# vmanam0451/distributed-path-tracer

Measured on AMD Instinct MI355X. Metric: Msamples/sec, Cornell box 1920x1080, 256 spp per frame, 8 bounces (camera paths traced per second), higher is better.
Workload: dtype f32

## Files before the change

distributed-path-tracer_amd/__init__.py:

```python
import atexit
import ctypes as C
import os
import re
import weakref

import numpy as np

_HERE = os.path.dirname(os.path.abspath(__file__))
LIB_PATH = os.environ.get("PTX_LIB") or os.path.join(_HERE, "libptx_hip.so")
HEADER_PATH = os.path.join(os.path.dirname(_HERE), "include", "ptx.h")

OK, ERR_INVALID, ERR_IO, ERR_PARSE, ERR_NO_CAMERA, ERR_NO_DEVICE, ERR_HIP, ERR_UNSUPPORTED = range(8)
NO_SUN_LIGHT = 0xFFFFFFFF

(ARR_MODEL_XFORM, ARR_MODEL_AABB, ARR_MODEL_SURF, ARR_SURF_RANGE, ARR_MESH_AABB, ARR_VERTICES, ARR_TRIANGLES,
 ARR_MATERIALS, ARR_KD_NODES, ARR_KD_REFS, ARR_CAMERA, ARR_SUN, ARR_MODEL_NAMES, ARR_TEXTURES, ARR_TEXELS, ARR_SURF_TEX, ARR_TEXELS_F32,
 ARR_LIGHT_TRIS, ARR_LIGHT_CDF, ARR_LIGHT_GEOM) = range(20)


class PtxError(RuntimeError):
    def __init__(self, code, msg):
        super().__init__(f"ptx error {code}: {msg}")
        self.code = code


class WorkItem(C.Structure):
    _fields_ = [("mesh_name", C.c_char_p), ("primitives", C.POINTER(C.c_int32)), ("n_primitives", C.c_uint32)]


class LoadOpts(C.Structure):
    _fields_ = [("camera_index", C.c_uint32), ("sun_light_index", C.c_uint32), ("filter_primitives", C.c_uint32),
                ("n_work", C.c_uint32), ("work", C.POINTER(WorkItem))]
# ... 217 lines not shown
    EXACT_MATH_FORMS = ("rcp", "sqrt", "rsqrt")

    def exact_math_check(self):
        out = np.zeros(len(self.EXACT_MATH_FORMS), np.uint64)
        _check(lib().ptx_exact_math_check(self.h, out.ctypes.data))
        return {n: int(v) for n, v in zip(self.EXACT_MATH_FORMS, out)}

    def leaf_intersect(self, corners, rays, refs=None, leaf_ordered=False):
        c = np.ascontiguousarray(corners, np.float32).reshape(-1, 9)
        r = np.ascontiguousarray(rays, np.float32).reshape(-1, 7)
        p = None if refs is None else np.ascontiguousarray(refs, np.uint32)
        if p is not None and p.shape != (len(c),):
            raise ValueError("refs must hold one reference per triangle")
        out = np.zeros((len(r), 3), np.float32)
        tri = np.full(len(r), -1, np.int32)
        _check(lib().ptx_leaf_intersect_batch(self.h, c.ctypes.data, len(c), None if p is None else p.ctypes.data, int(bool(leaf_ordered)),
                                              r.ctypes.data, len(r), out.ctypes.data, tri.ctypes.data))
        return {"t": out[:, 0].copy(), "beta": out[:, 1].copy(), "gamma": out[:, 2].copy(), "triangle": tri}

    def tonemap_encode(self, accum, W, H, spp, out=None):
        ret = out if out is not None else np.zeros((H, W, 4), np.uint8)
        _check(lib().ptx_tonemap_encode(self.h, _ptr(accum), W, H, spp, _ptr(ret)))
        return ret

    def denoise(self, a, b, albedo_cov, normal_depth, spp_a, spp_b, iterations=0, sigma_l=0, sigma_n=0, sigma_z=0, out=None, want_stats=True):
        bufs = [a, b, albedo_cov, normal_depth] + ([out] if out is not None else [])
        shape = tuple(a.shape)
        if len(shape) != 3 or shape[2] != 4 or any(tuple(x.shape) != shape for x in bufs):
            raise ValueError(f"denoise: every buffer must be [H, W, 4] of one size, got {[tuple(x.shape) for x in bufs]}")
        if out is None:
            out = np.empty(shape, np.float32) if isinstance(a, np.ndarray) else a.new_empty(shape)
# ... 29 lines not shown
            lib().ptx_ctx_destroy(self.h)
            self.h = None

    def __del__(self):
        try:
            self.close()
        except Exception:
            pass


_ARR_DTYPE = {ARR_MODEL_XFORM: (np.float32, 12), ARR_MODEL_AABB: (np.float32, 6), ARR_MODEL_SURF: (np.int32, 2),
              ARR_SURF_RANGE: (np.int32, 8), ARR_MESH_AABB: (np.float32, 6), ARR_VERTICES: (np.float32, 11),
              ARR_TRIANGLES: (np.uint32, 3), ARR_MATERIALS: (np.float32, 11), ARR_KD_NODES: (np.uint32, 2),
              ARR_KD_REFS: (np.uint32, 1), ARR_CAMERA: (np.float32, 1), ARR_SUN: (np.float32, 1),
              ARR_TEXTURES: (np.uint32, 4), ARR_TEXELS: (np.uint8, 1), ARR_SURF_TEX: (np.int32, 7), ARR_TEXELS_F32: (np.float32, 1),
              ARR_LIGHT_TRIS: (np.uint32, 2), ARR_LIGHT_CDF: (np.float32, 1), ARR_LIGHT_GEOM: (np.float32, 4)}


class Scene:

    def __init__(self, handle, ctx):
        self.h = handle
        self.ctx = ctx
        _live.add(self)

    @classmethod
    def load_gltf(cls, ctx, path, camera_index=0, sun_light_index=0, work=None):
        h = C.c_void_p()
        opts = LoadOpts(camera_index, sun_light_index, 0, 0, None)
        keep = []
        if work is not None:
# ... 281 lines not shown
```

distributed-path-tracer_amd/csrc/device_core.hpp:

```cpp
#pragma once
#include <hip/hip_runtime.h>
#include <stdint.h>
#include <stdlib.h>
#include <stdio.h>

#include "kernels.hpp"

namespace ptx {

#define DEV __device__ __forceinline__

#ifdef PTX_PROF
struct Prof { uint32_t t[kProfRegions], l[kProfRegions]; };
#define PROF_ARG , Prof& prof
#define PROF_PASS , prof
#define PROF(k) do { const uint64_t m_ = __ballot(true); prof.l[k] += 1u; prof.t[k] += ((threadIdx.x & 63u) == (uint32_t)(__ffsll((long long)m_) - 1)) ? 1u : 0u; } while (0)
#else
#define PROF_ARG
#define PROF_PASS
#define PROF(k) do { } while (0)
#endif

constexpr float kEps = 0.0001f;
constexpr double kPi = 3.14159265358979323846;
// ... 144 lines not shown
	if ((X.x > X.y) | (Y.x > Y.y) | (Z.x > Z.y)) return false;
	const f2 tx = (X - bc(o.x)) * bc(inv.x), ty = (Y - bc(o.y)) * bc(inv.y), tz = (Z - bc(o.z)) * bc(inv.z);
	const f2 sm = (tx + ty) + tz;
	const float s = sm.x + sm.y;
	if (s == s) {
		nr = hw_max3(hw_min(tx.x, tx.y), hw_min(ty.x, ty.y), hw_min(tz.x, tz.y));
		fr = hw_min3(hw_max(tx.x, tx.y), hw_max(ty.x, ty.y), hw_max(tz.x, tz.y));
	} else {
		nr = pmax(pmax(pmin(tx.x, tx.y), pmin(ty.x, ty.y)), pmin(tz.x, tz.y));
		fr = pmin(pmin(pmax(tx.x, tx.y), pmax(ty.x, ty.y)), pmax(tz.x, tz.y));
	}
	if (nr > fr) return false;
	return fr >= 0;
}

template <int PB>
DEV bool mesh_traverse(const Geom& g, uint32_t root, float nr, float fr, V3 o, V3 d, MeshHit& out, const Spill& spill PROF_ARG) {
	PROF(PB);
	const PRay pr = pack_ray(o, d);
	int sp = 0;
	uint32_t n0 = 0, n1 = 0, n2 = 0;
	float m0 = 0, m1 = 0, m2 = 0;
	uint32_t node = root;
	float min_dist = nr, max_dist = fr;
	bool have = true;
	for (;;) {
		PROF(PB + 1);
		if (!have) {
			if (sp == 0) return false;
			sp--;
// ... 42 lines not shown
				max_dist = split_dist;
			}
			if (!has_next) { valid = false; break; }
			node = next;
#ifdef PTX_LDS_PAIR_FETCH
			nd = pair_fetch ? (next == li ? kid0 : kid1) : g.nodes[node];
#else
			nd = (pair_fetch && g.pair) ? (next == li ? kid0 : kid1) : g.nodes[node];
#endif
		}
		if (!valid) continue;
		uint32_t first_ref = nd.x, count = nd.y >> 2;
		float best_t = -1.0f, bb1 = 0, bb2 = 0;
		uint32_t best_tri = 0;
		uint32_t key = 0;
		for (uint32_t i = 0; i < count; i++) {
			PROF(PB + 3);
			const uint32_t slot = g.leaf_ordered ? first_ref + i : g.refs[first_ref + i];
			const float4 r0 = g.tris[3 * slot], r1 = g.tris[3 * slot + 1], r2 = g.tris[3 * slot + 2];
			const uint32_t ti = __float_as_uint(r2.z);
			float be, ga;
			const float t = tri_test_pk<true>(r0, r1, make_float2(r2.x, r2.y), pr, be, ga, key);
			if (t >= 0 && t <= max_dist && (t < best_t || !(best_t >= 0))) { best_t = t; bb1 = be; bb2 = ga; best_tri = ti; }
		}
		if (key >= kRcpKeyEnd) {
			best_t = -1.0f; bb1 = 0; bb2 = 0; best_tri = 0;
			for (uint32_t i = 0; i < count; i++) {
				const uint32_t slot = g.leaf_ordered ? first_ref + i : g.refs[first_ref + i];
				const float4 r0 = g.tris[3 * slot], r1 = g.tris[3 * slot + 1], r2 = g.tris[3 * slot + 2];
				float be, ga;
				const float t = tri_test_pk<false>(r0, r1, make_float2(r2.x, r2.y), pr, be, ga, key);
				if (t >= 0 && t <= max_dist && (t < best_t || !(best_t >= 0))) { best_t = t; bb1 = be; bb2 = ga; best_tri = __float_as_uint(r2.z); }
			}
		}
		if (!(best_t >= 0)) continue;
		out.t = best_t; out.b1 = bb1; out.b2 = bb2; out.tri = best_tri;
		return true;
	}
}

template <int MODE, int PB>
DEV bool mesh_traverse_m(const Geoms& G, const SurfaceRec& sf, float nr, float fr, V3 o, V3 d, MeshHit& out, const Spill& spill PROF_ARG) {
	if constexpr (MODE == MODE_GLOBAL) return mesh_traverse<PB>(G.glb, sf.kd_root, nr, fr, o, d, out, spill PROF_PASS);
	else if constexpr (MODE == MODE_LDS) return mesh_traverse<PB>(G.lds, sf.lds_root, nr, fr, o, d, out, spill PROF_PASS);
	else {
		if (sf.lds_root != 0xFFFFFFFFu) return mesh_traverse<PB>(G.lds, sf.lds_root, nr, fr, o, d, out, spill PROF_PASS);
		return mesh_traverse<PB>(G.glb, sf.kd_root, nr, fr, o, d, out, spill PROF_PASS);
	}
}
template <int MODE, int PB>
DEV bool mesh_intersect_m(const Geoms& G, const SurfaceRec& sf, V3 o, V3 d, V3 inv, MeshHit& out, const Spill& spill PROF_ARG) {
	float nr, fr;
	if (!aabb_test_inv(sf.bmin, sf.bmax, o, inv, nr, fr)) return false;
	return mesh_traverse_m<MODE, PB>(G, sf, nr, fr, o, d, out, spill PROF_PASS);
}

struct SceneHit { float dist; int surface; uint32_t tri; float b1, b2; };

template <int MODE>
DEV bool scene_traverse(const DevScene& S, const Geoms& g, V3 o, V3 d, SceneHit& best, const Spill& spill) {
#ifdef PTX_PROF
// ... 519 lines not shown
```

distributed-path-tracer_amd/csrc/flat_scene.hpp:

```cpp
#pragma once
#include <cstdint>
#include <vector>
#include <string>

namespace ptx {

struct KdNode { uint32_t w0, w1; };
constexpr uint32_t KD_LEAF = 3u;
inline KdNode kd_make_branch(float split, uint32_t axis, bool has_l, bool has_r, uint32_t first_child) {
	uint32_t bits;
	__builtin_memcpy(&bits, &split, 4);
	return {bits, axis | (has_l ? 4u : 0u) | (has_r ? 8u : 0u) | (first_child << 4)};
}
inline KdNode kd_make_leaf(uint32_t first_ref, uint32_t count) { return {first_ref, KD_LEAF | (count << 2)}; }

struct TriRec { float ax, ay, az; uint32_t ia; float bx, by, bz; uint32_t ib; float cx, cy, cz; uint32_t ic; };

struct TriIsect { float e2y, e1z, e2z, e1y; float e1x, e2x, ay, az; float ax, c3, p0, p1; };
TriIsect make_tri_isect(const float* a, const float* b, const float* c, uint32_t gid);

struct HitRec { float a[3], ua, b[3], ub, c[3], uc, na[3], va, nb[3], vb, nc[3], vc, ta[3], p0, tb[3], p1, tc[3], p2; };
static_assert(sizeof(HitRec) == 144, "HitRec layout");

struct ModelRec {
// ... 8 lines not shown
	float pad0;
	float box[6], pbox[6];
};
static_assert(sizeof(ModelRec) == 60 * 4, "ModelRec layout");

struct SurfaceRec {
	float bmin[3], bmax[3];
	uint32_t kd_root;
	uint32_t tri_base;
	uint32_t lds_root;
	uint32_t model;
	float pbmin[3], pbmax[3];
	float box[6], pbox[6];
};
static_assert(sizeof(SurfaceRec) == 28 * 4, "SurfaceRec layout");
template <class Rec> inline void interleave_boxes(Rec& r) {
	for (int k = 0; k < 3; k++) { r.box[2 * k] = r.bmin[k]; r.box[2 * k + 1] = r.bmax[k]; r.pbox[2 * k] = r.pbmin[k]; r.pbox[2 * k + 1] = r.pbmax[k]; }
}

struct MaterialRec {
	float albedo[3]; float opacity;
	float emissive[3]; float roughness;
	float metallic; float ior; uint32_t shadow_catcher; uint32_t tex_mask;
	int32_t tex[7];
	int32_t pad;
};
static_assert(sizeof(MaterialRec) == 80, "MaterialRec layout");

struct TexRec { uint32_t w, h, c_srgb , offset ; };
constexpr uint32_t kTexSrgb = 1u << 8, kTexFloat = 1u << 16;
// ... 45 lines not shown
	SunRec sun{};
	uint32_t kd_max_depth = 0;
	bool any_texture = false;
	bool any_alpha = false;
	int32_t env_tex = -1;

	std::vector<KdNode> res_nodes;
	std::vector<uint32_t> res_refs;
	std::vector<TriIsect> res_tris;
	uint32_t n_resident = 0;
	size_t res_bytes = 0;

	size_t geometry_bytes() const { return kd_nodes.size() * 8 + kd_refs.size() * 4 + tris.size() * 48; }
};

void plan_residency(FlatScene& s, size_t lds_budget);

void finalize_scene(FlatScene& s, const float* camera13, const float* sun13);

struct Error {
	int code;
	std::string msg;
};
void read_png(const std::string& path, uint32_t& W, uint32_t& H, uint32_t& C, std::vector<uint8_t>& out);
void read_jpeg(const std::string& path, uint32_t& W, uint32_t& H, uint32_t& C, std::vector<uint8_t>& out);
bool is_hdr_file(const std::string& path);
void read_hdr(const std::string& path, uint32_t& W, uint32_t& H, uint32_t& C, std::vector<float>& out);
void read_image(const std::string& path, uint32_t& W, uint32_t& H, uint32_t& C, std::vector<uint8_t>& out);
TexRec load_texture(FlatScene& s, const std::string& path, bool srgb);
struct WorkFilter {
	bool filter = false;
// ... 14 lines not shown
```

distributed-path-tracer_amd/csrc/kernels.hip:

```cpp
#include <type_traits>

#include "device_core.hpp"

namespace ptx {

#ifdef PTX_CLK
#define CLK_T0() const uint64_t clk_t0_ = __builtin_amdgcn_s_memtime()
#define CLK_T1(k) do { clk[k] += __builtin_amdgcn_s_memtime() - clk_t0_; } while (0)
#define CLK_WAIT() __builtin_amdgcn_s_waitcnt(0)
#else
#define CLK_T0() do { } while (0)
#define CLK_T1(k) do { } while (0)
#define CLK_WAIT() do { } while (0)
#endif

template <int MODE, bool SUN, bool ALPHA, bool TEX, bool WORKER, bool SURF, bool TRANSP>
__global__ void __launch_bounds__(kBlock) k_render_pass(DevScene S0, RenderParams P, PassBuffers B, const ModelRec* __restrict__ t_models, const SurfaceRec* __restrict__ t_surfaces, const SpaceRec* __restrict__ t_spaces, const uint32_t* __restrict__ t_model_space) {
	DevScene S = S0;
	S.models = t_models; S.surfaces = t_surfaces; S.spaces = t_spaces; S.model_space = t_model_space;
	const Staged st = stage_geometry<MODE>(S, g_smem);
	S.hot_lds = st.hot;
	const Geoms g = st.g;
	const uint32_t lane = threadIdx.x & 63u;
	const uint32_t wave_slot = blockIdx.x * (kBlock / 64) + (threadIdx.x >> 6);
// ... 544 lines not shown
	q[0] = cone.x; q[1] = cone.y; q[2] = cone.z;
	q[3] = idf.x; q[4] = idf.y; q[5] = idf.z;
	q[6] = isp.x; q[7] = isp.y; q[8] = isp.z;
	q[9] = pdf_diffuse(nrm, inc);
	q[10] = pdf_specular(nrm, o, inc, rough);
	q[11] = fresnel_schlick(o, rf, ior);
	q[12] = rf.x; q[13] = rf.y; q[14] = rf.z;
}

__global__ void __launch_bounds__(256) k_leaf_intersect(const uint2* __restrict__ nodes, const uint32_t* __restrict__ refs, const float4* __restrict__ tris, uint32_t n_tri,
                                                        uint32_t leaf_ordered, const float* __restrict__ rays, size_t n, float* __restrict__ out, int32_t* __restrict__ tri,
                                                        uint2* __restrict__ spill_base) {
	__shared__ float4 s_tris[3 * kLeafBatchMaxTris];
	__shared__ uint32_t s_refs[kLeafBatchMaxTris];
	__shared__ uint2 s_node;
	if (!leaf_ordered) {
		for (uint32_t k = threadIdx.x; k < 3u * n_tri; k += blockDim.x) s_tris[k] = tris[k];
		for (uint32_t k = threadIdx.x; k < n_tri; k += blockDim.x) s_refs[k] = refs[k];
		if (threadIdx.x == 0) s_node = nodes[0];
		__syncthreads();
	}
	const Geom g = leaf_ordered ? Geom{nodes, refs, tris, true, true} : Geom{&s_node, s_refs, s_tris, false, false};
	const Spill spill{spill_base + (size_t)(blockIdx.x * (blockDim.x / 64) + (threadIdx.x >> 6)) * (kSpillStack * 64) + (threadIdx.x & 63u)};
#ifdef PTX_PROF
	Prof prof{};
#endif
	const size_t stride = (size_t)gridDim.x * blockDim.x;
	for (size_t i = (size_t)blockIdx.x * blockDim.x + threadIdx.x; i < n; i += stride) {
		const float* r = rays + 7 * i;
		MeshHit h;
		const bool hit = mesh_traverse<4>(g, 0u, 0.0f, r[6], mk(r[0], r[1], r[2]), mk(r[3], r[4], r[5]), h, spill PROF_PASS);
		out[3 * i] = hit ? h.t : -1.0f; out[3 * i + 1] = hit ? h.b1 : 0.0f; out[3 * i + 2] = hit ? h.b2 : 0.0f;
		tri[i] = hit ? (int32_t)h.tri : -1;
	}
}

DEV uint32_t differs(float u, float v) { return (__float_as_uint(u) != __float_as_uint(v) && !(u != u && v != v)) ? 1u : 0u; }
// ... 113 lines not shown
		hipError_t e = set_lds(reinterpret_cast<const void*>(&k_intersect_batch<MODE>), lds_bytes);
		if (e != hipSuccess) return e;
	}
	hipLaunchKernelGGL(k_intersect_batch<MODE>, dim3(grid), dim3(kBlock), MODE != MODE_GLOBAL ? lds_bytes : 0, stream, S, A, S.models, S.surfaces, S.spaces, S.model_space);
	return hipGetLastError();
}
hipError_t launch_intersect(const DevScene& S, const IntersectArgs& A, int mode, size_t lds_bytes, int grid, hipStream_t stream) {
	if (mode == MODE_LDS) return launch_intersect_mode<MODE_LDS>(S, A, lds_bytes, grid, stream);
	if (mode == MODE_HYBRID) return launch_intersect_mode<MODE_HYBRID>(S, A, lds_bytes, grid, stream);
	return launch_intersect_mode<MODE_GLOBAL>(S, A, lds_bytes, grid, stream);
}
hipError_t launch_pbr_eval(const float* in, float* out, size_t n, hipStream_t stream) {
	hipLaunchKernelGGL(k_pbr_eval, dim3((unsigned)((n + 255) / 256)), dim3(256), 0, stream, in, out, n);
	return hipGetLastError();
}
hipError_t launch_leaf_intersect(const uint2* nodes, const uint32_t* refs, const float4* tris, uint32_t n_tri, bool leaf_ordered, const float* rays, size_t n, float* out,
                                 int32_t* tri, uint2* spill, int grid, hipStream_t stream) {
	hipLaunchKernelGGL(k_leaf_intersect, dim3(grid), dim3(256), 0, stream, nodes, refs, tris, n_tri, leaf_ordered ? 1u : 0u, rays, n, out, tri, spill);
	return hipGetLastError();
}
hipError_t launch_exact_math_check(unsigned long long* bad, hipStream_t stream) {
	for (uint32_t form = 0; form < kExactMathForms; form++) {
		hipLaunchKernelGGL(k_exact_math_check, dim3(4096), dim3(256), 0, stream, form, bad);
		const hipError_t e = hipGetLastError();
		if (e != hipSuccess) return e;
	}
	return hipSuccess;
}
hipError_t launch_camera_rays(const DevScene& S, const float* in, float* out, size_t n, hipStream_t stream) {
	hipLaunchKernelGGL(k_camera_rays, dim3((unsigned)((n + 255) / 256)), dim3(256), 0, stream, S, in, out, n);
	return hipGetLastError();
}
hipError_t launch_material_eval(const DevScene& S, const int32_t* surface, const float* uv, size_t n, float* out, hipStream_t stream) {
// ... 10 lines not shown
```

distributed-path-tracer_amd/csrc/kernels.hpp:

```cpp
#pragma once
#include <hip/hip_runtime.h>
#include <cstdint>
#include <cstdlib>

#include "flat_scene.hpp"

namespace ptx {

#ifndef PTX_BLOCK
#define PTX_BLOCK 1024
#endif
constexpr int kBlock = PTX_BLOCK;
#ifndef PTX_CHUNK
#define PTX_CHUNK 2048
#endif
constexpr uint32_t kChunk = PTX_CHUNK;
#ifndef PTX_INLINE_MIN
#define PTX_INLINE_MIN 32
#endif
constexpr uint32_t kInlineMin = PTX_INLINE_MIN;
constexpr uint32_t kListCap = (kChunk / 64u) * (kInlineMin - 1u) + 16u;
constexpr int kMaxDeferModels = 64;
constexpr uint32_t kQueueFixedFloat4 = 12u * kChunk + kChunk / 2u;
inline uint32_t queue_float4_per_wave(uint32_t n_units) { return kQueueFixedFloat4 + (n_units <= (uint32_t)kMaxDeferModels ? n_units : 0u) * 2u * kListCap; }
// ... 103 lines not shown
constexpr int kWfMaxSurfaces = 64;
inline int wf_traverse_grid(int n_cu) { return n_cu * 8; }
hipError_t launch_wf_generate(const DevScene& S, const RenderParams& P, const WfStream& out, uint32_t cap, uint32_t first, uint32_t n, float4* sample_rad, hipStream_t stream);
hipError_t launch_wf_step(const DevScene& S, const RenderParams& P, const WfBuffers& W, const WfStream& in, const WfStream& out, uint32_t cap, uint32_t max_in,
                          uint32_t slab_first, uint32_t* n_out, float4* sample_rad, int n_cu, hipStream_t stream, hipEvent_t* ev );
hipError_t launch_wf_intersect(const DevScene& S, const IntersectArgs& A, size_t first_ray, uint32_t n, const WfBuffers& W, int n_cu, hipStream_t stream);

hipError_t launch_render_pass(const DevScene& S, const RenderParams& P, const PassBuffers& B, int mode, size_t lds_bytes, int grid,
                              hipStream_t stream);
hipError_t launch_resolve(const float4* sample_rad, float4* accum, const uint32_t* pixels, uint32_t n_pixels, uint32_t pass_spp, hipStream_t stream);
hipError_t launch_resolve_claim(const float4* sample_rad, float4* pixel_rgba, uint8_t* claimed, const uint32_t* pixels, uint32_t n_pixels, uint32_t pass_spp,
                                uint32_t sample0 , hipStream_t stream);
hipError_t launch_intersect(const DevScene& S, const IntersectArgs& A, int mode, size_t lds_bytes, int grid, hipStream_t stream);
hipError_t launch_pbr_eval(const float* in, float* out, size_t n, hipStream_t stream);
constexpr uint32_t kLeafBatchMaxTris = 256;
hipError_t launch_leaf_intersect(const uint2* nodes, const uint32_t* refs , const float4* tris , uint32_t n_tri, bool leaf_ordered,
                                 const float* rays , size_t n, float* out , int32_t* tri , uint2* spill, int grid, hipStream_t stream);
constexpr uint32_t kExactMathForms = 3;
hipError_t launch_exact_math_check(unsigned long long* bad , hipStream_t stream);
hipError_t launch_camera_rays(const DevScene& S, const float* in , float* out , size_t n, hipStream_t stream);
hipError_t launch_material_eval(const DevScene& S, const int32_t* surface , const float* uv , size_t n, float* out , hipStream_t stream);
hipError_t launch_tonemap(const float4* accum, uint32_t n_pixels, float spp, const float* thresholds , uchar4* out, hipStream_t stream);

struct AovStream {
	float *ox, *oy, *oz, *dx, *dy, *dz;
	uint32_t* id;
	uint32_t* pass;
};
struct AovHits {
	const int32_t *surface, *triangle;
	const float *b1, *b2;
// ... 61 lines not shown
```

distributed-path-tracer_amd/csrc/ptx_api.cpp:

```cpp
#include <dlfcn.h>
#include <hip/hip_runtime.h>
#include <zlib.h>

#include <algorithm>
#include <atomic>
#include <cstdio>
#include <cstdlib>
#include <cmath>
#include <cstring>
#include <mutex>
#include <string>
#include <vector>

#include "../../include/ptx.h"
#include "kernels.hpp"

using namespace ptx;

namespace {

thread_local std::string g_err;
int set_err(int code, const std::string& m) { g_err = m; return code; }
#define HIP_TRY(expr)                                                                                           \
	do {                                                                                                        \
// ... 63 lines not shown
	std::vector<hipEvent_t> step_events;
	ptx_kernel_timing timing{};
	uint32_t list_key[9] = {0, 0, 0, 0, 0, 0, 0, 0, 0};
	uint32_t list_len = 0;
};

struct ptx_scene {
	ptx_ctx* ctx = nullptr;
	FlatScene host;
	DevBuf d_models, d_surfaces, d_materials, d_nodes, d_refs, d_tris, d_shade, d_tex, d_texels, d_lut, d_spaces, d_model_space, d_wf_order;
	DevBuf d_res_nodes, d_res_refs, d_res_tris, d_texels_f, d_hot;
	DevScene dev{};
	double lds_area_share = 0;
	double wf_pairs_per_ray = 0;
	bool leaf_ordered = true;
	int mode = MODE_GLOBAL;
	size_t lds_bytes = 0;
	struct LightList {
		bool built = false, on_device = false;
		std::vector<uint32_t> tris;
		std::vector<float> cdf, geom;
		std::vector<int32_t> surf_first;
		float area = 0;
	} lights;
	std::mutex lights_mu;
	DevBuf d_light_tris, d_light_cdf, d_light_geom, d_light_first;
};

namespace {

size_t pad16(size_t b) { return (b + 15) & ~(size_t)15; }

void decide_mode(ptx_scene* sc) {
	FlatScene& h = sc->host;
	plan_residency(h, kLdsBudget);
	if (getenv("PTX_FORCE_GLOBAL") || h.n_resident == 0) sc->mode = MODE_GLOBAL;
	else if (h.n_resident == h.surfaces.size()) sc->mode = MODE_LDS;
	else sc->mode = getenv("PTX_NO_HYBRID") ? MODE_GLOBAL : MODE_HYBRID;
	if (sc->mode == MODE_GLOBAL) for (auto& sr : h.surfaces) sr.lds_root = 0xFFFFFFFFu;
	sc->lds_bytes = sc->mode == MODE_GLOBAL ? 0 : h.res_bytes;
	{
		double all = 0, res = 0;
		for (const SurfaceRec& sr : h.surfaces) {
			const double ex = sr.bmax[0] - sr.bmin[0], ey = sr.bmax[1] - sr.bmin[1], ez = sr.bmax[2] - sr.bmin[2];
			const double a = (ex > 0 && ey > 0 && ez > 0) ? 2 * (ex * ey + ey * ez + ex * ez) : 0;
			all += a;
			if (sr.lds_root != 0xFFFFFFFFu) res += a;
		}
		sc->lds_area_share = all > 0 ? res / all : 0;
	}
// ... 485 lines not shown
		tmp.push_back(h.camera.fov); tmp.push_back(h.camera.tan_half_fov);
		src = tmp.data(); bytes = tmp.size() * 4; break;
	case PTX_ARR_SUN:
		if (h.sun.present) { tmp.assign(h.sun.basis, h.sun.basis + 9); tmp.insert(tmp.end(), h.sun.energy, h.sun.energy + 3); tmp.push_back(h.sun.angular_radius); }
		src = tmp.data(); bytes = tmp.size() * 4; break;
	case PTX_ARR_MODEL_NAMES:
		for (auto& n : h.model_names) names += n + "\n";
		src = names.data(); bytes = names.size(); elem = 1; break;
	case PTX_ARR_TEXTURES: src = h.textures.data(); bytes = h.textures.size() * sizeof(TexRec); break;
	case PTX_ARR_TEXELS: src = h.texels.data(); bytes = h.texels.size(); elem = 1; break;
	case PTX_ARR_SURF_TEX: src = h.surf_tex.data(); bytes = h.surf_tex.size() * 4; break;
	case PTX_ARR_TEXELS_F32: src = h.texels_f.data(); bytes = h.texels_f.size() * 4; break;
	case PTX_ARR_LIGHT_TRIS: { const auto& ll = *build_lights(const_cast<ptx_scene*>(sc)); src = ll.tris.data(); bytes = ll.tris.size() * 4; break; }
	case PTX_ARR_LIGHT_CDF: { const auto& ll = *build_lights(const_cast<ptx_scene*>(sc)); src = ll.cdf.data(); bytes = ll.cdf.size() * 4; break; }
	case PTX_ARR_LIGHT_GEOM: { const auto& ll = *build_lights(const_cast<ptx_scene*>(sc)); src = ll.geom.data(); bytes = ll.geom.size() * 4; break; }
	default: set_err(PTX_ERR_INVALID, "unknown array id"); return -1;
	}
	if (dst) {
		if (dst_bytes < bytes) { set_err(PTX_ERR_INVALID, "destination too small"); return -1; }
		if (bytes) memcpy(dst, src, bytes);
	}
	return (int64_t)(bytes / elem);
}

namespace {

int32_t max_surfaces_per_model(const ptx_scene* sc) {
	int32_t m = 0;
	for (const ModelRec& mr : sc->host.models) m = std::max(m, mr.n_surfaces);
	return m;
// ... 1119 lines not shown
	const KdNode node[2] = {kd_make_leaf(0, n_tri), {0, 0}};
	std::lock_guard<std::mutex> lk(c->mu);
	HIP_TRY(hipSetDevice(c->device));
	const size_t refs_off = 16, recs_off = refs_off + pad16((size_t)n_tri * 4), rays_off = recs_off + (size_t)n_tri * 48;
	HIP_TRY(c->stage_a.ensure(rays_off + n * 28));
	HIP_TRY(c->stage_b.ensure(n * 16));
	char* in = (char*)c->stage_a.p;
	HIP_TRY(hipMemcpyAsync(in, node, 16, hipMemcpyHostToDevice, c->stream));
	HIP_TRY(hipMemcpyAsync(in + refs_off, order.data(), (size_t)n_tri * 4, hipMemcpyHostToDevice, c->stream));
	HIP_TRY(hipMemcpyAsync(in + recs_off, recs.data(), (size_t)n_tri * 48, hipMemcpyHostToDevice, c->stream));
	HIP_TRY(hipMemcpyAsync(in + rays_off, rays, n * 28, hipMemcpyHostToDevice, c->stream));
	const int grid = (int)std::min<size_t>((size_t)c->n_cu, (n + 255) / 256);
	HIP_TRY(c->spill.ensure((size_t)c->n_cu * 4 * (size_t)kSpillWords * sizeof(uint2)));
	float* d_out = (float*)c->stage_b.p;
	int32_t* d_tri = (int32_t*)(d_out + 3 * n);
	HIP_TRY(launch_leaf_intersect((const uint2*)in, (const uint32_t*)(in + refs_off), (const float4*)(in + recs_off), n_tri, leaf_ordered != 0,
	                              (const float*)(in + rays_off), n, d_out, d_tri, (uint2*)c->spill.p, grid, c->stream));
	HIP_TRY(hipMemcpyAsync(out, d_out, n * 12, hipMemcpyDeviceToHost, c->stream));
	HIP_TRY(hipMemcpyAsync(tri, d_tri, n * 4, hipMemcpyDeviceToHost, c->stream));
	HIP_TRY(hipStreamSynchronize(c->stream));
	return PTX_OK;
}

int ptx_exact_math_check(ptx_ctx* c, uint64_t* mismatches) {
	if (!c) return set_err(PTX_ERR_NO_DEVICE, "ptx_exact_math_check: no GPU context (no CPU path exists)");
	if (!mismatches) return set_err(PTX_ERR_INVALID, "ptx_exact_math_check: NULL argument");
	std::lock_guard<std::mutex> lk(c->mu);
	HIP_TRY(hipSetDevice(c->device));
	HIP_TRY(c->stage_b.ensure(kExactMathForms * 8));
	HIP_TRY(hipMemsetAsync(c->stage_b.p, 0, kExactMathForms * 8, c->stream));
	HIP_TRY(launch_exact_math_check((unsigned long long*)c->stage_b.p, c->stream));
// ... 154 lines not shown
```

distributed-path-tracer_amd/csrc/scene_build.cpp:

```cpp
#include "flat_scene.hpp"

#include <algorithm>
#include <cmath>
#include <cstdlib>
#include <cstring>
#include <deque>
#include <limits>
#include <atomic>
#include <exception>
#include <memory>
#include <mutex>
#include <thread>
#include <tuple>

namespace ptx {
namespace {

constexpr float kEps = 0.0001f;

struct F3 { float v[3]; };
struct Box { float lo[3], hi[3]; };

inline float pick_max(float a, float b) { return b > a ? b : a; }
inline float pick_min(float a, float b) { return b < a ? b : a; }
// ... 340 lines not shown
		}

	memcpy(s.camera.origin, cam, 12);
	memcpy(s.camera.basis, cam + 3, 36);
	s.camera.fov = cam[12];
	s.camera.tan_half_fov = std::tan(cam[12] * 0.5F);
	s.sun = SunRec{};
	if (sun) {
		memcpy(s.sun.basis, sun, 36);
		memcpy(s.sun.energy, sun + 9, 12);
		s.sun.angular_radius = sun[12];
		s.sun.present = 1;
	}
}

void plan_residency(FlatScene& s, size_t lds_budget) {
	const size_t n_surf = s.surfaces.size();
	s.res_nodes.clear(); s.res_refs.clear(); s.res_tris.clear();
	s.n_resident = 0;
	for (auto& sr : s.surfaces) sr.lds_root = 0xFFFFFFFFu;
	const size_t shade_bytes = s.shade.size() * sizeof(ShadeRec);
	auto bytes_of = [&](size_t si) {
		const int32_t* rg = &s.surf_range[8 * si];
		return (size_t)rg[5] * 8 + (size_t)rg[7] * 4 + (size_t)rg[3] * 48;
	};
	std::vector<size_t> order(n_surf);
	for (size_t i = 0; i < n_surf; i++) order[i] = i;
	std::stable_sort(order.begin(), order.end(), [&](size_t a, size_t b) { return bytes_of(a) < bytes_of(b); });
	std::vector<char> take(n_surf, 0);
	size_t used = shade_bytes + 48;
	for (size_t si : order) {
		if (used + bytes_of(si) > lds_budget) break;
		used += bytes_of(si);
		take[si] = 1;
	}
	for (size_t si = 0; si < n_surf; si++) {
		if (!take[si]) continue;
		const int32_t* rg = &s.surf_range[8 * si];
		const uint32_t t0 = (uint32_t)rg[2], nt = (uint32_t)rg[3], node0 = (uint32_t)rg[4], nn = (uint32_t)rg[5], ref0 = (uint32_t)rg[6], nr = (uint32_t)rg[7];
		const uint32_t nb = (uint32_t)s.res_nodes.size(), rb = (uint32_t)s.res_refs.size(), tb = (uint32_t)s.res_tris.size();
		for (uint32_t k = 0; k < nn; k++) {
			KdNode nd = s.kd_nodes[node0 + k];
			if ((nd.w1 & 3u) == KD_LEAF) nd.w0 = nd.w0 - ref0 + rb;
			else nd.w1 = (nd.w1 & 15u) | ((((nd.w1 >> 4) - node0) + nb) << 4);
			s.res_nodes.push_back(nd);
		}
		for (uint32_t k = 0; k < nr; k++) s.res_refs.push_back(s.kd_refs[ref0 + k] - t0 + tb);
		for (uint32_t k = 0; k < nt; k++) s.res_tris.push_back(s.tri_isect[t0 + k]);
		s.surfaces[si].lds_root = (s.surfaces[si].kd_root - node0) + nb;
		s.n_resident++;
	}
	s.res_bytes = s.res_tris.size() * 48 + shade_bytes + ((s.res_nodes.size() * 8 + 15) & ~(size_t)15) + ((s.res_refs.size() * 4 + 15) & ~(size_t)15);
}

}
```

include/ptx.h:

```cpp
#ifndef PTX_H
#define PTX_H

#include <stddef.h>
#include <stdint.h>

#ifdef __cplusplus
extern "C" {
#endif

typedef enum ptx_status {
	PTX_OK = 0,
	PTX_ERR_INVALID = 1,
	PTX_ERR_IO = 2,
	PTX_ERR_PARSE = 3,
	PTX_ERR_NO_CAMERA = 4,
	PTX_ERR_NO_DEVICE = 5,
	PTX_ERR_HIP = 6,
	PTX_ERR_UNSUPPORTED = 7
} ptx_status;

typedef struct ptx_ctx ptx_ctx;
typedef struct ptx_scene ptx_scene;

const char* ptx_last_error(void);
// ... 67 lines not shown
	PTX_ARR_MESH_AABB = 4,
	PTX_ARR_VERTICES = 5,
	PTX_ARR_TRIANGLES = 6,
	PTX_ARR_MATERIALS = 7,
	PTX_ARR_KD_NODES = 8,
	PTX_ARR_KD_REFS = 9,
	PTX_ARR_CAMERA = 10,
	PTX_ARR_SUN = 11,
	PTX_ARR_MODEL_NAMES = 12,
	PTX_ARR_TEXTURES = 13,
	PTX_ARR_TEXELS = 14,
	PTX_ARR_SURF_TEX = 15,
	PTX_ARR_TEXELS_F32 = 16,
	PTX_ARR_LIGHT_TRIS = 17,
	PTX_ARR_LIGHT_CDF = 18,
	PTX_ARR_LIGHT_GEOM = 19
} ptx_array;
int64_t ptx_scene_get_array(const ptx_scene* scene, ptx_array which, void* dst, size_t dst_bytes);

typedef enum ptx_integrator { PTX_INTEGRATOR_LIB = 0, PTX_INTEGRATOR_WORKER = 1 } ptx_integrator;
typedef struct ptx_render_cfg {
	uint32_t W, H;
	uint32_t spp;
	uint32_t bounces;
	float env[3];
	uint32_t seed_lo, seed_hi;
	uint32_t x0, y0, w, h;
	uint32_t sample0;
	uint32_t spp_per_pass;
	uint32_t integrator;
	uint32_t shard_index, shard_count, shard_tile;
// ... 103 lines not shown
```

Measured before the change: 1570.

## Store LDS-resident surfaces in leaf order to skip ref indirection

When planning LDS residency, surfaces whose triangle records can be duplicated into leaf order within a small extra byte cap are stored that way, and a flag bit on lds_root marks them. Traversal of those surfaces reads triangle records contiguously instead of going through a refs indirection in LDS, saving one LDS load per triangle test. The leaf loop is templated on the ordering so each path is branch-free per iteration. The cost is extra LDS bytes for duplicated triangles, which could reduce occupancy or push surfaces out of LDS, plus debug array exports and env knobs.

```diff
diff --git a/distributed-path-tracer_amd/__init__.py b/distributed-path-tracer_amd/__init__.py
--- a/distributed-path-tracer_amd/__init__.py
+++ b/distributed-path-tracer_amd/__init__.py
@@ -15,7 +15,9 @@
 
 (ARR_MODEL_XFORM, ARR_MODEL_AABB, ARR_MODEL_SURF, ARR_SURF_RANGE, ARR_MESH_AABB, ARR_VERTICES, ARR_TRIANGLES,
  ARR_MATERIALS, ARR_KD_NODES, ARR_KD_REFS, ARR_CAMERA, ARR_SUN, ARR_MODEL_NAMES, ARR_TEXTURES, ARR_TEXELS, ARR_SURF_TEX, ARR_TEXELS_F32,
- ARR_LIGHT_TRIS, ARR_LIGHT_CDF, ARR_LIGHT_GEOM) = range(20)
+ ARR_LIGHT_TRIS, ARR_LIGHT_CDF, ARR_LIGHT_GEOM, ARR_TRI_ISECT, ARR_RES_NODES, ARR_RES_REFS, ARR_RES_TRIS, ARR_LDS_ROOT,
+ ARR_RES_PLAN) = range(26)
+LDS_LEAF_ORDER_BIT = 0x80000000
 
 
 class PtxError(RuntimeError):
@@ -263,7 +265,7 @@
             raise ValueError("refs must hold one reference per triangle")
         out = np.zeros((len(r), 3), np.float32)
         tri = np.full(len(r), -1, np.int32)
-        _check(lib().ptx_leaf_intersect_batch(self.h, c.ctypes.data, len(c), None if p is None else p.ctypes.data, int(bool(leaf_ordered)),
+        _check(lib().ptx_leaf_intersect_batch(self.h, c.ctypes.data, len(c), None if p is None else p.ctypes.data, int(leaf_ordered),
                                               r.ctypes.data, len(r), out.ctypes.data, tri.ctypes.data))
         return {"t": out[:, 0].copy(), "beta": out[:, 1].copy(), "gamma": out[:, 2].copy(), "triangle": tri}
 
@@ -323,7 +325,9 @@
               ARR_TRIANGLES: (np.uint32, 3), ARR_MATERIALS: (np.float32, 11), ARR_KD_NODES: (np.uint32, 2),
               ARR_KD_REFS: (np.uint32, 1), ARR_CAMERA: (np.float32, 1), ARR_SUN: (np.float32, 1),
               ARR_TEXTURES: (np.uint32, 4), ARR_TEXELS: (np.uint8, 1), ARR_SURF_TEX: (np.int32, 7), ARR_TEXELS_F32: (np.float32, 1),
-              ARR_LIGHT_TRIS: (np.uint32, 2), ARR_LIGHT_CDF: (np.float32, 1), ARR_LIGHT_GEOM: (np.float32, 4)}
+              ARR_LIGHT_TRIS: (np.uint32, 2), ARR_LIGHT_CDF: (np.float32, 1), ARR_LIGHT_GEOM: (np.float32, 4),
+              ARR_TRI_ISECT: (np.uint32, 12), ARR_RES_NODES: (np.uint32, 2), ARR_RES_REFS: (np.uint32, 1), ARR_RES_TRIS: (np.uint32, 12),
+              ARR_LDS_ROOT: (np.uint32, 1), ARR_RES_PLAN: (np.uint32, 1)}
 
 
 class Scene:
diff --git a/distributed-path-tracer_amd/csrc/device_core.hpp b/distributed-path-tracer_amd/csrc/device_core.hpp
--- a/distributed-path-tracer_amd/csrc/device_core.hpp
+++ b/distributed-path-tracer_amd/csrc/device_core.hpp
@@ -182,6 +182,37 @@
 	return fr >= 0;
 }
 
+template <bool SHORT, bool LO>
+DEV void leaf_records(const Geom& g, uint32_t first, uint32_t count, const PRay& pr, float max_dist, float& best_t, float& bb1, float& bb2,
+                      uint32_t& best_tri, uint32_t& key) {
+	for (uint32_t i = 0; i < count; i++) {
+		const uint32_t slot = LO ? first + i : g.refs[first + i];
+		const float4 r0 = g.tris[3 * slot], r1 = g.tris[3 * slot + 1], r2 = g.tris[3 * slot + 2];
+		float be, ga;
+		const float t = tri_test_pk<SHORT>(r0, r1, make_float2(r2.x, r2.y), pr, be, ga, key);
+		if (t >= 0 && t <= max_dist && (t < best_t || !(best_t >= 0))) { best_t = t; bb1 = be; bb2 = ga; best_tri = __float_as_uint(r2.z); }
+	}
+}
+template <bool SHORT, int PB>
+DEV void leaf_trip(const Geom& g, uint32_t first, uint32_t count, const PRay& pr, float max_dist, float& best_t, float& bb1, float& bb2,
+                   uint32_t& best_tri, uint32_t& key PROF_ARG) {
+#ifdef PTX_PROF
+	if (SHORT) for (uint32_t i = 0; i < count; i++) PROF(PB + 3);
+#endif
+#ifdef PTX_LEAF_ONE_LOOP
+	for (uint32_t i = 0; i < count; i++) {
+		const uint32_t slot = g.leaf_ordered ? first + i : g.refs[first + i];
+		const float4 r0 = g.tris[3 * slot], r1 = g.tris[3 * slot + 1], r2 = g.tris[3 * slot + 2];
+		float be, ga;
+		const float t = tri_test_pk<SHORT>(r0, r1, make_float2(r2.x, r2.y), pr, be, ga, key);
+		if (t >= 0 && t <= max_dist && (t < best_t || !(best_t >= 0))) { best_t = t; bb1 = be; bb2 = ga; best_tri = __float_as_uint(r2.z); }
+	}
+#else
+	if (g.leaf_ordered) leaf_records<SHORT, true>(g, first, count, pr, max_dist, best_t, bb1, bb2, best_tri, key);
+	else leaf_records<SHORT, false>(g, first, count, pr, max_dist, best_t, bb1, bb2, best_tri, key);
+#endif
+}
+
 template <int PB>
 DEV bool mesh_traverse(const Geom& g, uint32_t root, float nr, float fr, V3 o, V3 d, MeshHit& out, const Spill& spill PROF_ARG) {
 	PROF(PB);
@@ -254,24 +285,10 @@
 		float best_t = -1.0f, bb1 = 0, bb2 = 0;
 		uint32_t best_tri = 0;
 		uint32_t key = 0;
-		for (uint32_t i = 0; i < count; i++) {
-			PROF(PB + 3);
-			const uint32_t slot = g.leaf_ordered ? first_ref + i : g.refs[first_ref + i];
-			const float4 r0 = g.tris[3 * slot], r1 = g.tris[3 * slot + 1], r2 = g.tris[3 * slot + 2];
-			const uint32_t ti = __float_as_uint(r2.z);
-			float be, ga;
-			const float t = tri_test_pk<true>(r0, r1, make_float2(r2.x, r2.y), pr, be, ga, key);
-			if (t >= 0 && t <= max_dist && (t < best_t || !(best_t >= 0))) { best_t = t; bb1 = be; bb2 = ga; best_tri = ti; }
-		}
+		leaf_trip<true, PB>(g, first_ref, count, pr, max_dist, best_t, bb1, bb2, best_tri, key PROF_PASS);
 		if (key >= kRcpKeyEnd) {
 			best_t = -1.0f; bb1 = 0; bb2 = 0; best_tri = 0;
-			for (uint32_t i = 0; i < count; i++) {
-				const uint32_t slot = g.leaf_ordered ? first_ref + i : g.refs[first_ref + i];
-				const float4 r0 = g.tris[3 * slot], r1 = g.tris[3 * slot + 1], r2 = g.tris[3 * slot + 2];
-				float be, ga;
-				const float t = tri_test_pk<false>(r0, r1, make_float2(r2.x, r2.y), pr, be, ga, key);
-				if (t >= 0 && t <= max_dist && (t < best_t || !(best_t >= 0))) { best_t = t; bb1 = be; bb2 = ga; best_tri = __float_as_uint(r2.z); }
-			}
+			leaf_trip<false, PB>(g, first_ref, count, pr, max_dist, best_t, bb1, bb2, best_tri, key PROF_PASS);
 		}
 		if (!(best_t >= 0)) continue;
 		out.t = best_t; out.b1 = bb1; out.b2 = bb2; out.tri = best_tri;
@@ -279,12 +296,13 @@
 	}
 }
 
+DEV Geom lds_geom(const Geom& lds, uint32_t lds_root) { return {lds.nodes, lds.refs, lds.tris, (lds_root & kLdsLeafOrderBit) != 0, lds.pair}; }
 template <int MODE, int PB>
 DEV bool mesh_traverse_m(const Geoms& G, const SurfaceRec& sf, float nr, float fr, V3 o, V3 d, MeshHit& out, const Spill& spill PROF_ARG) {
 	if constexpr (MODE == MODE_GLOBAL) return mesh_traverse<PB>(G.glb, sf.kd_root, nr, fr, o, d, out, spill PROF_PASS);
-	else if constexpr (MODE == MODE_LDS) return mesh_traverse<PB>(G.lds, sf.lds_root, nr, fr, o, d, out, spill PROF_PASS);
+	else if constexpr (MODE == MODE_LDS) return mesh_traverse<PB>(lds_geom(G.lds, sf.lds_root), sf.lds_root & ~kLdsLeafOrderBit, nr, fr, o, d, out, spill PROF_PASS);
 	else {
-		if (sf.lds_root != 0xFFFFFFFFu) return mesh_traverse<PB>(G.lds, sf.lds_root, nr, fr, o, d, out, spill PROF_PASS);
+		if (sf.lds_root != 0xFFFFFFFFu) return mesh_traverse<PB>(lds_geom(G.lds, sf.lds_root), sf.lds_root & ~kLdsLeafOrderBit, nr, fr, o, d, out, spill PROF_PASS);
 		return mesh_traverse<PB>(G.glb, sf.kd_root, nr, fr, o, d, out, spill PROF_PASS);
 	}
 }
diff --git a/distributed-path-tracer_amd/csrc/flat_scene.hpp b/distributed-path-tracer_amd/csrc/flat_scene.hpp
--- a/distributed-path-tracer_amd/csrc/flat_scene.hpp
+++ b/distributed-path-tracer_amd/csrc/flat_scene.hpp
@@ -46,6 +46,7 @@
 	float box[6], pbox[6];
 };
 static_assert(sizeof(SurfaceRec) == 28 * 4, "SurfaceRec layout");
+constexpr uint32_t kLdsLeafOrderBit = 0x80000000u;
 template <class Rec> inline void interleave_boxes(Rec& r) {
 	for (int k = 0; k < 3; k++) { r.box[2 * k] = r.bmin[k]; r.box[2 * k + 1] = r.bmax[k]; r.pbox[2 * k] = r.pbmin[k]; r.pbox[2 * k + 1] = r.pbmax[k]; }
 }
@@ -121,7 +122,8 @@
 	size_t geometry_bytes() const { return kd_nodes.size() * 8 + kd_refs.size() * 4 + tris.size() * 48; }
 };
 
-void plan_residency(FlatScene& s, size_t lds_budget);
+constexpr size_t kLdsLeafOrderCap = 4096;
+void plan_residency(FlatScene& s, size_t lds_budget, bool lds_leaf_order = true);
 
 void finalize_scene(FlatScene& s, const float* camera13, const float* sun13);
 
diff --git a/distributed-path-tracer_amd/csrc/kernels.hip b/distributed-path-tracer_amd/csrc/kernels.hip
--- a/distributed-path-tracer_amd/csrc/kernels.hip
+++ b/distributed-path-tracer_amd/csrc/kernels.hip
@@ -582,13 +582,13 @@
 	__shared__ float4 s_tris[3 * kLeafBatchMaxTris];
 	__shared__ uint32_t s_refs[kLeafBatchMaxTris];
 	__shared__ uint2 s_node;
-	if (!leaf_ordered) {
+	if (leaf_ordered != 1u) {
 		for (uint32_t k = threadIdx.x; k < 3u * n_tri; k += blockDim.x) s_tris[k] = tris[k];
-		for (uint32_t k = threadIdx.x; k < n_tri; k += blockDim.x) s_refs[k] = refs[k];
+		if (!leaf_ordered) for (uint32_t k = threadIdx.x; k < n_tri; k += blockDim.x) s_refs[k] = refs[k];
 		if (threadIdx.x == 0) s_node = nodes[0];
 		__syncthreads();
 	}
-	const Geom g = leaf_ordered ? Geom{nodes, refs, tris, true, true} : Geom{&s_node, s_refs, s_tris, false, false};
+	const Geom g = leaf_ordered == 1u ? Geom{nodes, refs, tris, true, true} : Geom{&s_node, s_refs, s_tris, leaf_ordered == 2u, false};
 	const Spill spill{spill_base + (size_t)(blockIdx.x * (blockDim.x / 64) + (threadIdx.x >> 6)) * (kSpillStack * 64) + (threadIdx.x & 63u)};
 #ifdef PTX_PROF
 	Prof prof{};
@@ -732,9 +732,9 @@
 	hipLaunchKernelGGL(k_pbr_eval, dim3((unsigned)((n + 255) / 256)), dim3(256), 0, stream, in, out, n);
 	return hipGetLastError();
 }
-hipError_t launch_leaf_intersect(const uint2* nodes, const uint32_t* refs, const float4* tris, uint32_t n_tri, bool leaf_ordered, const float* rays, size_t n, float* out,
+hipError_t launch_leaf_intersect(const uint2* nodes, const uint32_t* refs, const float4* tris, uint32_t n_tri, uint32_t leaf_ordered, const float* rays, size_t n, float* out,
                                  int32_t* tri, uint2* spill, int grid, hipStream_t stream) {
-	hipLaunchKernelGGL(k_leaf_intersect, dim3(grid), dim3(256), 0, stream, nodes, refs, tris, n_tri, leaf_ordered ? 1u : 0u, rays, n, out, tri, spill);
+	hipLaunchKernelGGL(k_leaf_intersect, dim3(grid), dim3(256), 0, stream, nodes, refs, tris, n_tri, leaf_ordered, rays, n, out, tri, spill);
 	return hipGetLastError();
 }
 hipError_t launch_exact_math_check(unsigned long long* bad, hipStream_t stream) {
diff --git a/distributed-path-tracer_amd/csrc/kernels.hpp b/distributed-path-tracer_amd/csrc/kernels.hpp
--- a/distributed-path-tracer_amd/csrc/kernels.hpp
+++ b/distributed-path-tracer_amd/csrc/kernels.hpp
@@ -141,7 +141,7 @@
 hipError_t launch_intersect(const DevScene& S, const IntersectArgs& A, int mode, size_t lds_bytes, int grid, hipStream_t stream);
 hipError_t launch_pbr_eval(const float* in, float* out, size_t n, hipStream_t stream);
 constexpr uint32_t kLeafBatchMaxTris = 256;
-hipError_t launch_leaf_intersect(const uint2* nodes, const uint32_t* refs , const float4* tris , uint32_t n_tri, bool leaf_ordered,
+hipError_t launch_leaf_intersect(const uint2* nodes, const uint32_t* refs , const float4* tris , uint32_t n_tri, uint32_t leaf_ordered ,
                                  const float* rays , size_t n, float* out , int32_t* tri , uint2* spill, int grid, hipStream_t stream);
 constexpr uint32_t kExactMathForms = 3;
 hipError_t launch_exact_math_check(unsigned long long* bad , hipStream_t stream);
diff --git a/distributed-path-tracer_amd/csrc/ptx_api.cpp b/distributed-path-tracer_amd/csrc/ptx_api.cpp
--- a/distributed-path-tracer_amd/csrc/ptx_api.cpp
+++ b/distributed-path-tracer_amd/csrc/ptx_api.cpp
@@ -101,6 +101,8 @@
 	double lds_area_share = 0;
 	double wf_pairs_per_ray = 0;
 	bool leaf_ordered = true;
+	int lds_leaf_order = -1;
+	size_t lds_budget = 0;
 	int mode = MODE_GLOBAL;
 	size_t lds_bytes = 0;
 	struct LightList {
@@ -120,7 +122,13 @@
 
 void decide_mode(ptx_scene* sc) {
 	FlatScene& h = sc->host;
-	plan_residency(h, kLdsBudget);
+	if (sc->lds_leaf_order < 0) {
+		const char* e = getenv("PTX_LDS_LEAF_ORDER");
+		sc->lds_leaf_order = (e && e[0] == '0') ? 0 : 1;
+		sc->lds_budget = kLdsBudget;
+		if (const char* b = getenv("PTX_LDS_BUDGET")) sc->lds_budget = std::min<size_t>(kLdsBudget, (size_t)strtoull(b, nullptr, 10));
+	}
+	plan_residency(h, sc->lds_budget, sc->lds_leaf_order != 0);
 	if (getenv("PTX_FORCE_GLOBAL") || h.n_resident == 0) sc->mode = MODE_GLOBAL;
 	else if (h.n_resident == h.surfaces.size()) sc->mode = MODE_LDS;
 	else sc->mode = getenv("PTX_NO_HYBRID") ? MODE_GLOBAL : MODE_HYBRID;
@@ -636,6 +644,18 @@
 	case PTX_ARR_LIGHT_TRIS: { const auto& ll = *build_lights(const_cast<ptx_scene*>(sc)); src = ll.tris.data(); bytes = ll.tris.size() * 4; break; }
 	case PTX_ARR_LIGHT_CDF: { const auto& ll = *build_lights(const_cast<ptx_scene*>(sc)); src = ll.cdf.data(); bytes = ll.cdf.size() * 4; break; }
 	case PTX_ARR_LIGHT_GEOM: { const auto& ll = *build_lights(const_cast<ptx_scene*>(sc)); src = ll.geom.data(); bytes = ll.geom.size() * 4; break; }
+	case PTX_ARR_TRI_ISECT: src = h.tri_isect.data(); bytes = h.tri_isect.size() * sizeof(TriIsect); break;
+	case PTX_ARR_RES_NODES: src = h.res_nodes.data(); bytes = h.res_nodes.size() * 8; break;
+	case PTX_ARR_RES_REFS: src = h.res_refs.data(); bytes = h.res_refs.size() * 4; break;
+	case PTX_ARR_RES_TRIS: src = h.res_tris.data(); bytes = h.res_tris.size() * sizeof(TriIsect); break;
+	case PTX_ARR_LDS_ROOT:
+		for (auto& s : h.surfaces) { float f; memcpy(&f, &s.lds_root, 4); tmp.push_back(f); }
+		src = tmp.data(); bytes = tmp.size() * 4; break;
+	case PTX_ARR_RES_PLAN: {
+		const uint32_t w[4] = {(uint32_t)h.res_bytes, h.n_resident, (uint32_t)sc->lds_bytes, (uint32_t)h.hot_hitrec.size()};
+		tmp.resize(4); memcpy(tmp.data(), w, 16);
+		src = tmp.data(); bytes = 16; break;
+	}
 	default: set_err(PTX_ERR_INVALID, "unknown array id"); return -1;
 	}
 	if (dst) {
@@ -1785,7 +1805,7 @@
 	HIP_TRY(c->spill.ensure((size_t)c->n_cu * 4 * (size_t)kSpillWords * sizeof(uint2)));
 	float* d_out = (float*)c->stage_b.p;
 	int32_t* d_tri = (int32_t*)(d_out + 3 * n);
-	HIP_TRY(launch_leaf_intersect((const uint2*)in, (const uint32_t*)(in + refs_off), (const float4*)(in + recs_off), n_tri, leaf_ordered != 0,
+	HIP_TRY(launch_leaf_intersect((const uint2*)in, (const uint32_t*)(in + refs_off), (const float4*)(in + recs_off), n_tri, leaf_ordered == 0 ? 0u : (leaf_ordered == 2 ? 2u : 1u),
 	                              (const float*)(in + rays_off), n, d_out, d_tri, (uint2*)c->spill.p, grid, c->stream));
 	HIP_TRY(hipMemcpyAsync(out, d_out, n * 12, hipMemcpyDeviceToHost, c->stream));
 	HIP_TRY(hipMemcpyAsync(tri, d_tri, n * 4, hipMemcpyDeviceToHost, c->stream));
diff --git a/distributed-path-tracer_amd/csrc/scene_build.cpp b/distributed-path-tracer_amd/csrc/scene_build.cpp
--- a/distributed-path-tracer_amd/csrc/scene_build.cpp
+++ b/distributed-path-tracer_amd/csrc/scene_build.cpp
@@ -1,6 +1,7 @@
 #include "flat_scene.hpp"
 
 #include <algorithm>
+#include <cassert>
 #include <cmath>
 #include <cstdlib>
 #include <cstring>
@@ -378,7 +379,7 @@
 	}
 }
 
-void plan_residency(FlatScene& s, size_t lds_budget) {
+void plan_residency(FlatScene& s, size_t lds_budget, bool lds_leaf_order) {
 	const size_t n_surf = s.surfaces.size();
 	s.res_nodes.clear(); s.res_refs.clear(); s.res_tris.clear();
 	s.n_resident = 0;
@@ -398,6 +399,26 @@
 		used += bytes_of(si);
 		take[si] = 1;
 	}
+	std::vector<char> leaf_order(n_surf, 0);
+	if (lds_leaf_order) {
+		auto extra_of = [&](size_t si) {
+			const int32_t* rg = &s.surf_range[8 * si];
+			return ((int64_t)rg[7] - rg[3]) * 48 - (int64_t)rg[7] * 4;
+		};
+		std::vector<size_t> cand;
+		for (size_t si = 0; si < n_surf; si++) if (take[si]) cand.push_back(si);
+		std::stable_sort(cand.begin(), cand.end(), [&](size_t a, size_t b) { return extra_of(a) < extra_of(b); });
+		const int64_t cap = (int64_t)std::min(kLdsLeafOrderCap, lds_budget > used ? lds_budget - used : (size_t)0);
+		int64_t spent = 0;
+		for (size_t si : cand) {
+			const int64_t e = extra_of(si);
+			if (e > 0) {
+				if (spent + e > cap) break;
+				spent += e;
+			}
+			leaf_order[si] = 1;
+		}
+	}
 	for (size_t si = 0; si < n_surf; si++) {
 		if (!take[si]) continue;
 		const int32_t* rg = &s.surf_range[8 * si];
@@ -405,13 +426,19 @@
 		const uint32_t nb = (uint32_t)s.res_nodes.size(), rb = (uint32_t)s.res_refs.size(), tb = (uint32_t)s.res_tris.size();
 		for (uint32_t k = 0; k < nn; k++) {
 			KdNode nd = s.kd_nodes[node0 + k];
-			if ((nd.w1 & 3u) == KD_LEAF) nd.w0 = nd.w0 - ref0 + rb;
+			if ((nd.w1 & 3u) == KD_LEAF) nd.w0 = nd.w0 - ref0 + (leaf_order[si] ? tb : rb);
 			else nd.w1 = (nd.w1 & 15u) | ((((nd.w1 >> 4) - node0) + nb) << 4);
 			s.res_nodes.push_back(nd);
 		}
-		for (uint32_t k = 0; k < nr; k++) s.res_refs.push_back(s.kd_refs[ref0 + k] - t0 + tb);
-		for (uint32_t k = 0; k < nt; k++) s.res_tris.push_back(s.tri_isect[t0 + k]);
-		s.surfaces[si].lds_root = (s.surfaces[si].kd_root - node0) + nb;
+		if (leaf_order[si]) {
+			for (uint32_t k = 0; k < nr; k++) s.res_tris.push_back(s.tri_isect[s.kd_refs[ref0 + k]]);
+		} else {
+			for (uint32_t k = 0; k < nr; k++) s.res_refs.push_back(s.kd_refs[ref0 + k] - t0 + tb);
+			for (uint32_t k = 0; k < nt; k++) s.res_tris.push_back(s.tri_isect[t0 + k]);
+		}
+		const uint32_t root = (s.surfaces[si].kd_root - node0) + nb;
+		assert(root < kLdsLeafOrderBit);
+		s.surfaces[si].lds_root = root | (leaf_order[si] ? kLdsLeafOrderBit : 0u);
 		s.n_resident++;
 	}
 	s.res_bytes = s.res_tris.size() * 48 + shade_bytes + ((s.res_nodes.size() * 8 + 15) & ~(size_t)15) + ((s.res_refs.size() * 4 + 15) & ~(size_t)15);
diff --git a/include/ptx.h b/include/ptx.h
--- a/include/ptx.h
+++ b/include/ptx.h
@@ -105,7 +105,13 @@
 	PTX_ARR_TEXELS_F32 = 16,
 	PTX_ARR_LIGHT_TRIS = 17,
 	PTX_ARR_LIGHT_CDF = 18,
-	PTX_ARR_LIGHT_GEOM = 19
+	PTX_ARR_LIGHT_GEOM = 19,
+	PTX_ARR_TRI_ISECT = 20,
+	PTX_ARR_RES_NODES = 21,
+	PTX_ARR_RES_REFS = 22,
+	PTX_ARR_RES_TRIS = 23,
+	PTX_ARR_LDS_ROOT = 24,
+	PTX_ARR_RES_PLAN = 25
 } ptx_array;
 int64_t ptx_scene_get_array(const ptx_scene* scene, ptx_array which, void* dst, size_t dst_bytes);
 
```

After: 1594, median of 6. 1.02x the previous value.
